# ndlongvn/MM-DTI

Measured on AMD Instinct MI355X. Metric: molecules/sec fwd+bwd (InfoNCE fine-tune), higher is better.
Workload: dtype fp16 forward / bf16 backward GEMM operands, fp32 accumulation

## Files before the change

### mm-dti_amd/csrc/pair_attn.h

```cpp
#pragma once
#include <type_traits>

#include "common.h"

namespace mmdti {

constexpr int HD = 8;

__device__ __forceinline__ void load8_bf16(const bf16_t* p, float (&o)[8]) {
  uint4 u = *reinterpret_cast<const uint4*>(p);
  uint32_t w[4] = {u.x, u.y, u.z, u.w};
#pragma unroll
  for (int i = 0; i < 4; ++i) {
    o[2 * i] = __uint_as_float(w[i] << 16);
    o[2 * i + 1] = __uint_as_float(w[i] & 0xffff0000u);
  }
}
__device__ __forceinline__ void store8_bf16(bf16_t* p, const float (&v)[8]) {
  uint4 u;
  u.x = (uint32_t)f2bf(v[0]) | ((uint32_t)f2bf(v[1]) << 16);
  u.y = (uint32_t)f2bf(v[2]) | ((uint32_t)f2bf(v[3]) << 16);
  u.z = (uint32_t)f2bf(v[4]) | ((uint32_t)f2bf(v[5]) << 16);
  u.w = (uint32_t)f2bf(v[6]) | ((uint32_t)f2bf(v[7]) << 16);
  *reinterpret_cast<uint4*>(p) = u;
}


typedef float f32x4 __attribute__((ext_vector_type(4)));

typedef short pa_s16x4 __attribute__((ext_vector_type(4)));
typedef __bf16 pa_bf16x4 __attribute__((ext_vector_type(4)));
typedef __attribute__((address_space(3))) pa_s16x4 pa_lds_s16x4;

__device__ __forceinline__ pa_s16x4 pa_pack4(const f32x4& v) {
  pa_bf16x4 h;
  h[0] = (__bf16)v[0]; h[1] = (__bf16)v[1]; h[2] = (__bf16)v[2]; h[3] = (__bf16)v[3];
  return __builtin_bit_cast(pa_s16x4, h);
}
__device__ __forceinline__ void pa_split4(const f32x4& v, pa_s16x4& hi, pa_s16x4& lo) {
  pa_bf16x4 h;
  h[0] = (__bf16)v[0]; h[1] = (__bf16)v[1]; h[2] = (__bf16)v[2]; h[3] = (__bf16)v[3];
  f32x4 r;
  r[0] = v[0] - (float)h[0]; r[1] = v[1] - (float)h[1]; r[2] = v[2] - (float)h[2]; r[3] = v[3] - (float)h[3];
  hi = __builtin_bit_cast(pa_s16x4, h);
  lo = pa_pack4(r);
}
#define PA_MFMA16(A, B, C) __builtin_amdgcn_mfma_f32_16x16x16bf16_1k(A, B, C, 0, 0, 0)
typedef _Float16 pa_h16x4 __attribute__((ext_vector_type(4)));
template <bool F16>
__device__ __forceinline__ f32x4 pa_mfma16(const pa_s16x4& a, const pa_s16x4& b, const f32x4& c) {
  if constexpr (F16) return __builtin_amdgcn_mfma_f32_16x16x16f16(__builtin_bit_cast(pa_h16x4, a), __builtin_bit_cast(pa_h16x4, b), c, 0, 0, 0);
  else return __builtin_amdgcn_mfma_f32_16x16x16bf16_1k(a, b, c, 0, 0, 0);
}
template <bool F16>
__device__ __forceinline__ void pa_split4_t(const f32x4& v, pa_s16x4& hi, pa_s16x4& lo) {
  if constexpr (F16) {
    pa_h16x4 h, l;
#pragma unroll
    for (int r = 0; r < 4; ++r) {
      h[r] = (_Float16)v[r];
      l[r] = (_Float16)(v[r] - (float)h[r]);
    }
    hi = __builtin_bit_cast(pa_s16x4, h);
    lo = __builtin_bit_cast(pa_s16x4, l);
  } else {
    pa_split4(v, hi, lo);
  }
}
#define PA_LOG2E 1.44269504088896340736f

typedef _Float16 pa_f16x4 __attribute__((ext_vector_type(4)));
__device__ __forceinline__ f32x4 pa_load4(const float* p) { return *reinterpret_cast<const f32x4*>(p); }
__device__ __forceinline__ f32x4 pa_load4_nt(const float* p) { return __builtin_nontemporal_load(reinterpret_cast<const f32x4*>(p)); }
__device__ __forceinline__ void pa_store4_nt(float* p, f32x4 v) { __builtin_nontemporal_store(v, reinterpret_cast<f32x4*>(p)); }
__device__ __forceinline__ f32x4 pa_round4(f32x4& keep, f32x4 v) { keep = v; return v; }

__device__ __forceinline__ f32x4 pa_widen_f16(const pa_f16x4& h) {
  f32x4 v;
#pragma unroll
  for (int r = 0; r < 4; ++r) v[r] = (float)h[r];
  return v;
}
__device__ __forceinline__ pa_f16x4 pa_narrow_f16(const f32x4& v) {
  pa_f16x4 h;
#pragma unroll
  for (int r = 0; r < 4; ++r) h[r] = (_Float16)v[r];
  return h;
}
__device__ __forceinline__ f32x4 pa_load4(const _Float16* p) { return pa_widen_f16(*reinterpret_cast<const pa_f16x4*>(p)); }
__device__ __forceinline__ f32x4 pa_load4_nt(const _Float16* p) { return pa_widen_f16(__builtin_nontemporal_load(reinterpret_cast<const pa_f16x4*>(p))); }
__device__ __forceinline__ void pa_store4_nt(_Float16* p, const f32x4& v) {
  __builtin_nontemporal_store(pa_narrow_f16(v), reinterpret_cast<pa_f16x4*>(p));
}
__device__ __forceinline__ f32x4 pa_round4(pa_f16x4& keep, const f32x4& v) {
  f32x4 c;
#pragma unroll
  for (int r = 0; r < 4; ++r) c[r] = __builtin_amdgcn_fmed3f(v[r], -INFINITY, 65504.f);
  keep = pa_narrow_f16(c);
  return pa_widen_f16(keep);
}
__device__ __forceinline__ void pa_store4_nt(_Float16* p, const pa_f16x4& h) { __builtin_nontemporal_store(h, reinterpret_cast<pa_f16x4*>(p)); }

__device__ __forceinline__ f32x4 pa_widen_bf16(const pa_s16x4& h) {
  f32x4 v;
#pragma unroll
  for (int r = 0; r < 4; ++r) v[r] = __builtin_bit_cast(float, (uint32_t)(uint16_t)h[r] << 16);
  return v;
}
__device__ __forceinline__ f32x4 pa_load4(const __bf16* p) { return pa_widen_bf16(*reinterpret_cast<const pa_s16x4*>(p)); }
__device__ __forceinline__ f32x4 pa_load4_nt(const __bf16* p) { return pa_widen_bf16(__builtin_nontemporal_load(reinterpret_cast<const pa_s16x4*>(p))); }
__device__ __forceinline__ void pa_store4_nt(__bf16* p, const f32x4& v) { __builtin_nontemporal_store(pa_pack4(v), reinterpret_cast<pa_s16x4*>(p)); }

__host__ __device__ constexpr int pa_kt_step(int nt) { return nt <= 9 ? 1 : (nt <= 13 ? 2 : 4); }
__host__ __device__ constexpr int pa_kt_effective(int kt, int nt) {
  const int s = pa_kt_step(nt), k = ((kt < 1 ? 1 : kt) + s - 1) / s * s;
  return k >= nt ? nt : k;
}
template <int NT, int K, typename F>
__device__ __forceinline__ void pa_dispatch_kt(int ke, F&& f) {
  constexpr int step = pa_kt_step(NT);
  constexpr int below = (K == NT) ? ((NT - 1) / step) * step : K - step;
  if constexpr (below < 1) {
    f(std::integral_constant<int, K>{});
  } else {
    if (ke >= K) f(std::integral_constant<int, K>{});
    else pa_dispatch_kt<NT, below>(ke, f);
  }
}

}

#define PA_MAX_NT 17

static inline int check_common(const char* fn, int B, int N, int H, int ld) {
  MMDTI_REQUIRE(B > 0 && N > 0 && H > 0, "%s: B,N,H must be positive", fn);
  MMDTI_REQUIRE(N <= 320, "%s: N=%d exceeds the supported 320 atoms (+BOS/EOS)", fn, N);
  MMDTI_REQUIRE(ld >= N, "%s: ld (%d) < N (%d)", fn, ld, N);
  MMDTI_REQUIRE((long long)B * H <= 2147483647LL, "%s: grid too large", fn);
  return MMDTI_OK;
}
```

### mm-dti_amd/csrc/pair_attn.hip

```cpp
#include "pair_attn.h"

namespace mmdti {

template <int NCH>
__global__ __launch_bounds__(256) void pair_attn_fwd_kernel(const bf16_t* __restrict__ qkv,
                                                            const float* __restrict__ bias_in,
                                                            float* __restrict__ s_out, bf16_t* __restrict__ o,
                                                            const unsigned char* __restrict__ key_pad, int N, int H,
                                                            int ld, float scale, uint32_t thresh, float dscale,
                                                            uint64_t seed, uint32_t site) {
  __shared__ __attribute__((aligned(16))) float sq[NCH * 64][HD];
  const int bh = xcd_chunk(blockIdx.x, gridDim.x), b = bh / H, h = bh - b * H;
  const int D = H * HD, D3 = 3 * D;
  const int tid = threadIdx.x, lane = tid & 63, wave = tid >> 6;
  const bf16_t* base = qkv + (long long)b * N * D3 + h * HD;
  for (int t = tid; t < N; t += 256) {
    float q[8];
    load8_bf16(base + (long long)t * D3, q);
#pragma unroll
    for (int d = 0; d < 8; ++d) sq[t][d] = q[d];
  }
  float k[NCH][8], v[NCH][8];
  bool masked[NCH];
#pragma unroll
  for (int c = 0; c < NCH; ++c) {
    const int j = c * 64 + lane;
    masked[c] = true;
#pragma unroll
    for (int d = 0; d < 8; ++d) k[c][d] = v[c][d] = 0.f;
    if (j < N) {
      load8_bf16(base + (long long)j * D3 + D, k[c]);
      load8_bf16(base + (long long)j * D3 + 2 * D, v[c]);
      masked[c] = key_pad ? key_pad[b * N + j] != 0 : false;
    }
  }
  __syncthreads();
  const float NEG_INF = -INFINITY;
  float nb[NCH];
#pragma unroll
  for (int c = 0; c < NCH; ++c) {
    const int j = c * 64 + lane;
    nb[c] = (wave < N && j < N && !masked[c]) ? bias_in[((long long)bh * N + wave) * ld + j] : 0.f;
  }
  for (int i = wave; i < N; i += 4) {
    const float4 q0 = *reinterpret_cast<const float4*>(&sq[i][0]);
    const float4 q1 = *reinterpret_cast<const float4*>(&sq[i][4]);
    const long long rowoff = ((long long)bh * N + i) * ld;
    float cb[NCH];
#pragma unroll
    for (int c = 0; c < NCH; ++c) cb[c] = nb[c];
    if (i + 4 < N) {
#pragma unroll
      for (int c = 0; c < NCH; ++c) {
        const int j = c * 64 + lane;
        nb[c] = (j < N && !masked[c]) ? bias_in[rowoff + 4LL * ld + j] : 0.f;
      }
    }
    float sv[NCH];
    float m = NEG_INF;
#pragma unroll
    for (int c = 0; c < NCH; ++c) {
      const int j = c * 64 + lane;
      float s = NEG_INF;
      if (j < N) {
        float dot = q0.x * k[c][0] + q0.y * k[c][1] + q0.z * k[c][2] + q0.w * k[c][3] + q1.x * k[c][4] +
                    q1.y * k[c][5] + q1.z * k[c][6] + q1.w * k[c][7];
        s = masked[c] ? NEG_INF : scale * dot + cb[c];
        s_out[rowoff + j] = s;
      }
      sv[c] = s;
      m = fmaxf(m, s);
    }
    m = wave_max(m);
    float sum = 0.f;
#pragma unroll
    for (int c = 0; c < NCH; ++c) {
      sv[c] = __expf(sv[c] - m);
      sum += sv[c];
    }
    const float inv = 1.0f / wave_sum(sum);
    float acc[8] = {0.f, 0.f, 0.f, 0.f, 0.f, 0.f, 0.f, 0.f};
#pragma unroll
    for (int c = 0; c < NCH; ++c) {
      float p = sv[c] * inv;
      if (thresh) {
        const int j = c * 64 + lane;
        bool keep = dropout_keep(seed, site, ((uint64_t)bh * N + i) * ld + j, thresh);
        p = keep ? p * dscale : 0.f;
      }
#pragma unroll
      for (int d = 0; d < 8; ++d) acc[d] += p * v[c][d];
    }
    const float tot = wave_sum8_scatter(acc, lane);
    if (lane < 8) o[((long long)b * N + i) * D + h * HD + lane] = f2bf(tot);
  }
}

template <int NT, bool TILED, bool FULL, bool RAG, typename ST, bool F16 = false>
__global__ __launch_bounds__(256, NT > 9 ? 2 : 4) void pair_attn_fwd_mfma_kernel(const bf16_t* __restrict__ qkv, const ST* __restrict__ bias_in,
                                                                 ST* __restrict__ s_out, bf16_t* __restrict__ o,
                                                                 const unsigned char* __restrict__ key_pad, int N, int H, int ld,
                                                                 float scale, uint32_t thresh, float dscale, uint64_t seed,
                                                                 uint32_t site, const int* __restrict__ key_tiles, int rag_store,
                                                                 const int* __restrict__ row_off) {
  static_assert(TILED || sizeof(ST) == 4, "compact pair tensors exist in the tiled layout only");
  static_assert(!RAG || sizeof(ST) == 2, "key-tile skipping is built for the compact layout only");
  constexpr int NP = NT * 16;
  constexpr int KSTR = NP + 8;
  __shared__ __attribute__((aligned(16))) bf16_t sQ[NP * 8];
  __shared__ __attribute__((aligned(16))) bf16_t sK[NP * 8];
  __shared__ __attribute__((aligned(16))) bf16_t sVT[8 * KSTR];
  __shared__ __attribute__((aligned(16))) float sM[NP];
  const int bh = xcd_chunk(blockIdx.x, gridDim.x), b = bh / H, h = bh - b * H;
  const int D = H * HD, D3 = 3 * D;
  const int tid = threadIdx.x, lane = tid & 63, wave = tid >> 6, nwaves = blockDim.x >> 6;
  const int nKB = (N + 15) >> 4;
  const int kt = RAG ? pa_kt_effective(min(__builtin_amdgcn_readfirstlane(key_tiles[b]), nKB), NT) : NT;
  const bool packed = RAG && row_off != nullptr;
  const int row0 = packed ? __builtin_amdgcn_readfirstlane(row_off[b]) : b * N;
  const int rows = packed ? __builtin_amdgcn_readfirstlane(row_off[b + 1]) - row0 : N;
  const bf16_t* base = qkv + (long long)row0 * D3 + h * HD;
  for (int t = tid; t < NP; t += blockDim.x) {
    uint4 q = make_uint4(0u, 0u, 0u, 0u), kk = q, vv = q;
    float msk = 1.f;
    if (t < rows) {
      q = *reinterpret_cast<const uint4*>(base + (long long)t * D3);
      kk = *reinterpret_cast<const uint4*>(base + (long long)t * D3 + D);
      vv = *reinterpret_cast<const uint4*>(base + (long long)t * D3 + 2 * D);
      msk = (key_pad && key_pad[row0 + t]) ? 1.f : 0.f;
    }
    *reinterpret_cast<uint4*>(sQ + t * 8) = q;
    *reinterpret_cast<uint4*>(sK + t * 8) = kk;
    const uint32_t vw[4] = {vv.x, vv.y, vv.z, vv.w};
#pragma unroll
    for (int d = 0; d < 8; ++d) sVT[d * KSTR + t] = (bf16_t)((d & 1) ? (vw[d >> 1] >> 16) : (vw[d >> 1] & 0xffffu));
    sM[t] = msk;
  }
  for (int t = tid; t < 8 * 8; t += blockDim.x) sVT[(t >> 3) * KSTR + NP + (t & 7)] = 0;
  __syncthreads();
  const int g = lane >> 4, c16 = lane & 15;
  const float NEG_INF = -INFINITY;
  const int nlast = nKB - 1;
  const bool colok = 4 * g < N - 16 * nlast;
  const Rng24 rk = rng24_key(seed, site, (uint32_t)bh);
  auto body = [&](int qb, auto edge_c, auto kt_c) {
    constexpr bool EDGE = decltype(edge_c)::value;
    constexpr int KT = decltype(kt_c)::value;
    const int qi = qb * 16 + c16;
    const uint32_t t8 = thresh ? rng24_row_t8(rk, (uint32_t)qi, thresh) : 0u;
    const bool qvalid = EDGE ? qi < rows : true;
    const long long rowoff = ((long long)bh * N + (qvalid ? qi : 0)) * ld;
    const pa_s16x4 zero4 = {0, 0, 0, 0};
    const pa_s16x4 qv = g < 2 ? *reinterpret_cast<const pa_s16x4*>(sQ + (qb * 16 + c16) * 8 + 4 * g) : zero4;
    const int vr = EDGE ? min(16, N - qb * 16) : 16;
    const long long tbase = (long long)bh * pair_plane(N) + (long long)qb * 16 * pair_n4(N) + ((4 * g < pair_n4(N) ? g : 0) * vr + (qvalid ? c16 : 0)) * 4;
    const ST* bin = bias_in + (TILED ? tbase : rowoff);
    ST* sout = s_out + (TILED ? tbase : rowoff);
    const int TSTEP = TILED ? (EDGE ? vr * 16 : 256) : 16;
    const int goff = TILED ? 0 : 4 * g;
#define PA_PRED(T) (!TILED ? (qvalid && (T) * 16 + 4 * g < N) \
                           : (qvalid && (FULL ? ((T) < NT - 1 || colok) : ((T) < nlast || ((T) == nlast && colok)))))
#define PA_FAST(T) (TILED && !EDGE && (FULL ? (T) < NT - 1 : false))
    const float fillv = (TILED && qvalid) ? -INFINITY : 0.f;
    f32x4 S[KT];
#pragma unroll
    for (int t = 0; t < KT; ++t) {
      if (PA_FAST(t)) {
        S[t] = pa_load4_nt(bin + t * TSTEP + goff);
      } else {
        const bool pr = PA_PRED(t);
        const f32x4 ld4 = pa_load4(bin + (pr ? t * TSTEP + goff : 0));
        S[t] = pr ? ld4 : f32x4{fillv, fillv, fillv, fillv};
      }
    }
    float m = NEG_INF;
    if (RAG && rag_store) {
      const f32x4 ninf = {NEG_INF, NEG_INF, NEG_INF, NEG_INF};
#pragma unroll
      for (int t = KT; t < NT; ++t) {
        if (PA_FAST(t)) {
          pa_store4_nt(sout + t * TSTEP + goff, ninf);
        } else if (PA_PRED(t)) {
          pa_store4_nt(sout + t * TSTEP + goff, ninf);
        }
      }
    }
#pragma unroll
    for (int t = 0; t < KT; ++t) {
      {
        const int kcol = t * 16 + 4 * g;
        f32x4 c = S[t];
        const pa_s16x4 ka = g < 2 ? *reinterpret_cast<const pa_s16x4*>(sK + (t * 16 + c16) * 8 + 4 * g) : zero4;
        f32x4 qk = {0.f, 0.f, 0.f, 0.f};
        qk = pa_mfma16<F16>(ka, qv, qk);
#pragma unroll
        for (int r = 0; r < 4; ++r) c[r] += scale * qk[r];
        if (!TILED || key_pad) {
          const f32x4 km = *reinterpret_cast<const f32x4*>(&sM[kcol]);
#pragma unroll
          for (int r = 0; r < 4; ++r) c[r] = (km[r] != 0.f) ? NEG_INF : c[r];
        }
        typename std::conditional<sizeof(ST) == 2, pa_f16x4, f32x4>::type cs;
        c = pa_round4(cs, c);
        if (PA_FAST(t)) {
          pa_store4_nt(sout + t * TSTEP + goff, cs);
        } else if (PA_PRED(t)) {
          pa_store4_nt(sout + t * TSTEP + goff, cs);
        }
        S[t] = c;
        m = fmaxf(fmaxf(m, c[0]), c[1]);
        m = fmaxf(fmaxf(m, c[2]), c[3]);
      }
    }
    m = fmaxf(m, __shfl_xor(m, 16, 64));
    m = fmaxf(m, __shfl_xor(m, 32, 64));
    const float mneg = -m * PA_LOG2E;
    float lsum = 0.f;
#pragma unroll
    for (int t = 0; t < KT; ++t) {
      {
#pragma unroll
        for (int r = 0; r < 4; ++r) {
          const float e = __builtin_amdgcn_exp2f(fmaf(S[t][r], PA_LOG2E, mneg));
          S[t][r] = e;
          lsum += e;
        }
      }
    }
    lsum += __shfl_xor(lsum, 16, 64);
    lsum += __shfl_xor(lsum, 32, 64);
    const float inv = dscale / lsum;
    f32x4 oacc = {0.f, 0.f, 0.f, 0.f};
#pragma unroll
    for (int t = 0; t < KT; ++t) {
      {
        f32x4 p = S[t] * inv;
        if (thresh) {
          const uint32_t kw = rng24_word(rk, ((uint32_t)qi * (uint32_t)ld + t * 16 + 4 * g) >> 2);
#pragma unroll
          for (int r = 0; r < 4; ++r) p[r] = rng24_kept(kw, r, t8) ? p[r] : 0.f;
        }
        const pa_s16x4 va = *reinterpret_cast<const pa_s16x4*>(sVT + (c16 & 7) * KSTR + t * 16 + 4 * g);
        pa_s16x4 ph, pl;
        pa_split4_t<F16>(p, ph, pl);
        oacc = pa_mfma16<F16>(va, ph, oacc);
        oacc = pa_mfma16<F16>(va, pl, oacc);
      }
    }
    if (qvalid && g < 2) {
      uint2 pk;
      if constexpr (F16) {
        pk.x = f2h_sat2(oacc[0], oacc[1]);
        pk.y = f2h_sat2(oacc[2], oacc[3]);
      } else {
        pk.x = (uint32_t)f2bf(oacc[0]) | ((uint32_t)f2bf(oacc[1]) << 16);
        pk.y = (uint32_t)f2bf(oacc[2]) | ((uint32_t)f2bf(oacc[3]) << 16);
      }
      *reinterpret_cast<uint2*>(o + ((long long)row0 + qi) * D + h * HD + 4 * g) = pk;
    }
#undef PA_PRED
#undef PA_FAST
  };
  const int nQB = packed ? (rows + 15) >> 4 : nKB;
  auto run = [&](auto kt_c) {
    for (int qb = wave; qb < nQB; qb += nwaves) {
      if (TILED && qb * 16 + 16 <= rows) body(qb, std::false_type{}, kt_c);
      else body(qb, std::true_type{}, kt_c);
    }
  };
  if constexpr (RAG) pa_dispatch_kt<NT, NT>(kt, run);
  else run(std::integral_constant<int, NT>{});
}


}
MMDTI_DEFINE_SALT_PULL(pair_attn)
using namespace mmdti;

extern "C" int mmdti_pair_attn_fwd(mmdti_stream_t stream, const void* qkv_bf16, const void* bias_in, void* s_out,
                                   void* o_bf16, const unsigned char* key_pad, int B, int N, int H, int ld,
                                   float scale, float drop_p, unsigned long long seed, unsigned int site, int layout,
                                   const int* key_tiles, int rag_store, const int* row_off, int qkv_f16) {
  const int tiled = layout & 1, compact = (layout >> 1) & 1;
  if (int e = check_common("pair_attn_fwd", B, N, H, ld)) return e;
  MMDTI_REQUIRE((layout & ~3) == 0 && (!compact || tiled), "pair_attn_fwd: layout must be 0 (row-major fp32), 1 (tiled fp32) or 3 (tiled, fp16 logits)");
  MMDTI_REQUIRE(!key_tiles || compact, "pair_attn_fwd: key_tiles (ragged batches) needs the compact tiled pair layout (layout 3)");
  MMDTI_REQUIRE(!row_off || key_tiles, "pair_attn_fwd: packed token rows (row_off) need key_tiles");
  MMDTI_REQUIRE(!qkv_f16 || compact, "pair_attn_fwd: fp16 q | k | v (the fp16 forward-operand mode) is built for the compact tiled pair layout (layout 3)");
  MMDTI_REQUIRE(!tiled || (ld % 4 == 0 && N <= 16 * PA_MAX_NT), "pair_attn_fwd: the tiled pair layout needs ld %% 4 == 0 and N <= 272");
  MMDTI_REQUIRE(qkv_bf16 && bias_in && s_out && o_bf16, "pair_attn_fwd: null pointer");
  MMDTI_REQUIRE(aligned16(qkv_bf16), "pair_attn_fwd: qkv must be 16-byte aligned");
  MMDTI_REQUIRE(!tiled || (aligned16(bias_in) && aligned16(s_out)), "pair_attn_fwd: tiled pair tensors must be 16-byte aligned");
  MMDTI_REQUIRE(drop_p >= 0.f && drop_p < 1.f, "pair_attn_fwd: dropout p out of range");
  const uint32_t th = dropout_thresh(drop_p);
  const uint32_t th8 = dropout_thresh8(drop_p);
  const float sc = drop_p > 0.f ? 1.f / (1.f - drop_p) : 1.f;
  dim3 grid(B * H), block(256);
  hipStream_t s = (hipStream_t)stream;
  if (ld % 4 == 0 && aligned16(bias_in) && aligned16(s_out) && N <= 16 * PA_MAX_NT) {
    const int nqb = (N + 15) / 16;
    dim3 blk(nqb % 3 == 0 ? 192 : (nqb < 4 ? 64 * nqb : 256));
#define PA_M(NT, TL, FL, RG, ST)                                                                                                     \
  hipLaunchKernelGGL((pair_attn_fwd_mfma_kernel<NT, TL, FL, RG, ST>), grid, blk, 0, s, (const bf16_t*)qkv_bf16, (const ST*)bias_in, \
                     (ST*)s_out, (bf16_t*)o_bf16, key_pad, N, H, ld, scale, th8, sc, (uint64_t)seed, (uint32_t)site, key_tiles, rag_store, row_off)
#define PA_MT(NT)                                                                           \
  do {                                                                                      \
    if (!tiled) PA_M(NT, false, false, false, float);                                       \
    else if (!compact) { if (nqb == NT) PA_M(NT, true, true, false, float); else PA_M(NT, true, false, false, float); } \
  } while (0)
#define PA_MH(NT, RG)                                                                                                                  \
  hipLaunchKernelGGL((pair_attn_fwd_mfma_kernel<NT, true, true, RG, _Float16, true>), grid, blk, 0, s, (const bf16_t*)qkv_bf16,       \
                     (const _Float16*)bias_in, (_Float16*)s_out, (bf16_t*)o_bf16, key_pad, N, H, ld, scale, th8, sc, (uint64_t)seed,  \
                     (uint32_t)site, key_tiles, rag_store, row_off)
#define PA_MC(NT) case NT: if (qkv_f16) { if (key_tiles) PA_MH(NT, true); else PA_MH(NT, false); } \
                           else if (key_tiles) PA_M(NT, true, true, true, _Float16); else PA_M(NT, true, true, false, _Float16); break
    if (compact) {
      switch (nqb) {
        PA_MC(1); PA_MC(2); PA_MC(3); PA_MC(4); PA_MC(5); PA_MC(6); PA_MC(7); PA_MC(8); PA_MC(9); PA_MC(10); PA_MC(11); PA_MC(12);
        PA_MC(13); PA_MC(14); PA_MC(15); PA_MC(16); PA_MC(17);
      }
    } else if (nqb <= 5) PA_MT(5); else if (nqb <= 9) PA_MT(9); else if (nqb <= 13) PA_MT(13); else PA_MT(17);
#undef PA_MC
#undef PA_MH
#undef PA_MT
#undef PA_M
    MMDTI_LAUNCH_CHECK();
    return MMDTI_OK;
  }
#define PA_F(NCH)                                                                                                   \
  hipLaunchKernelGGL((pair_attn_fwd_kernel<NCH>), grid, block, 0, s, (const bf16_t*)qkv_bf16, (const float*)bias_in, (float*)s_out, \
                     (bf16_t*)o_bf16, key_pad, N, H, ld, scale, th, sc, (uint64_t)seed, (uint32_t)site)
  switch ((N + 63) / 64) {
    case 1: PA_F(1); break;
    case 2: PA_F(2); break;
    case 3: PA_F(3); break;
    case 4: PA_F(4); break;
    default: PA_F(5); break;
  }
#undef PA_F
  MMDTI_LAUNCH_CHECK();
  return MMDTI_OK;
}
```

### mm-dti_amd/csrc/pair_attn_bwd_mfma.h

```cpp
#pragma once
#include "pair_attn.h"

namespace mmdti {

template <int NT, bool TILED, bool FULL, int NW, bool RAG, typename ST, typename GT>
__global__ __launch_bounds__(64 * NW, NT > 9 ? ((NT >= 16 && NW == 3) ? 2 : 1) : 3) void pair_attn_bwd_mfma_kernel(const bf16_t* __restrict__ qkv, const ST* __restrict__ s_in,
                                                                 const bf16_t* __restrict__ dO, const GT* __restrict__ gin, GT* __restrict__ gout,
                                                                 bf16_t* __restrict__ dqkv, int N, int H, int ld, float scale,
                                                                 int g_in_zero, uint32_t thresh, float dscale, uint64_t seed,
                                                                 uint32_t site, const int* __restrict__ key_tiles,
                                                                 const int* __restrict__ row_off, int qkv_f16) {
  static_assert(TILED || (sizeof(ST) == 4 && sizeof(GT) == 4), "compact pair tensors exist in the tiled layout only");
  static_assert(!RAG || sizeof(ST) == 2, "key-tile skipping is built for the compact layout only");
  constexpr int NP = NT * 16;
  constexpr int KSTR = NP + 8;
  __shared__ __attribute__((aligned(16))) bf16_t sQ[NP * 8 + 16];
  __shared__ __attribute__((aligned(16))) bf16_t sD[NP * 8 + 16];
  __shared__ __attribute__((aligned(16))) bf16_t sV[NP * 8];
  __shared__ __attribute__((aligned(16))) bf16_t sKT[8 * KSTR];
  __shared__ __attribute__((aligned(16))) float redw[NW * NT * 2 * 128];
  __shared__ __attribute__((aligned(16))) bf16_t patch[NW][2][256];
  const int bh = xcd_chunk(blockIdx.x, gridDim.x), b = bh / H, h = bh - b * H;
  const int D = H * HD, D3 = 3 * D;
  const int tid = threadIdx.x, lane = tid & 63, wave = tid >> 6, nwaves = blockDim.x >> 6;
  const int nKB = (N + 15) >> 4;
  const int kt = RAG ? pa_kt_effective(min(__builtin_amdgcn_readfirstlane(key_tiles[b]), nKB), NT) : NT;
  const bool packed = RAG && row_off != nullptr;
  const int row0 = packed ? __builtin_amdgcn_readfirstlane(row_off[b]) : b * N;
  const int rows = packed ? __builtin_amdgcn_readfirstlane(row_off[b + 1]) - row0 : N;
  const bf16_t* base = qkv + (long long)row0 * D3 + h * HD;
  for (int t = tid; t < NP + 2; t += blockDim.x) {
    uint4 q = make_uint4(0u, 0u, 0u, 0u), kk = q, vv = q, dd = q;
    if (t < rows) {
      q = *reinterpret_cast<const uint4*>(base + (long long)t * D3);
      kk = *reinterpret_cast<const uint4*>(base + (long long)t * D3 + D);
      vv = *reinterpret_cast<const uint4*>(base + (long long)t * D3 + 2 * D);
      dd = *reinterpret_cast<const uint4*>(dO + ((long long)row0 + t) * D + h * HD);
      if (qkv_f16) { q = h2bf8(q); kk = h2bf8(kk); vv = h2bf8(vv); }
    }
    *reinterpret_cast<uint4*>(sQ + t * 8) = q;
    *reinterpret_cast<uint4*>(sD + t * 8) = dd;
    if (t < NP) {
      *reinterpret_cast<uint4*>(sV + t * 8) = vv;
      const uint32_t kw[4] = {kk.x, kk.y, kk.z, kk.w};
#pragma unroll
      for (int d = 0; d < 8; ++d) sKT[d * KSTR + t] = (bf16_t)((d & 1) ? (kw[d >> 1] >> 16) : (kw[d >> 1] & 0xffffu));
    }
  }
  for (int t = tid; t < 8 * 8; t += blockDim.x) sKT[(t >> 3) * KSTR + NP + (t & 7)] = 0;
  for (int t = tid; t < NW * NT * 2 * 128; t += blockDim.x) redw[t] = 0.f;
  __syncthreads();
  const int g = lane >> 4, c16 = lane & 15;
  const bool dlane = c16 < 8;
  const float NEG_INF = -INFINITY;
  bf16_t* pw = &patch[wave][0][0];
  const int pwr = c16 * 16 + ((g ^ ((c16 >> 3) << 1)) << 2);
  const int prd = (4 * g + (c16 >> 2)) * 16 + (((c16 & 3) ^ ((g >> 1) << 1)) << 2);
  const pa_s16x4 zero4 = {0, 0, 0, 0};
  const int nlast = nKB - 1;
  const bool colok = 4 * g < N - 16 * nlast;
  const Rng24 rk = rng24_key(seed, site, (uint32_t)bh);
  auto body = [&](int qb, auto edge_c, auto kt_c) {
    constexpr bool EDGE = decltype(edge_c)::value;
    constexpr int KT = decltype(kt_c)::value;
    const int qi = qb * 16 + c16;
    const uint32_t t8 = thresh ? rng24_row_t8(rk, (uint32_t)qi, thresh) : 0u;
    const bool qvalid = EDGE ? qi < rows : true;
    const long long rowoff = ((long long)bh * N + (qvalid ? qi : 0)) * ld;
    const int vr = EDGE ? min(16, N - qb * 16) : 16;
    const long long tbase = (long long)bh * pair_plane(N) + (long long)qb * 16 * pair_n4(N) + ((4 * g < pair_n4(N) ? g : 0) * vr + (qvalid ? c16 : 0)) * 4;
    const ST* sin_p = s_in + (TILED ? tbase : rowoff);
    const GT* gin_p = gin + (TILED ? tbase : rowoff);
    GT* gout_p = gout + (TILED ? tbase : rowoff);
    const int TSTEP = TILED ? (EDGE ? vr * 16 : 256) : 16;
    const int goff = TILED ? 0 : 4 * g;
#define PA_PRED(T) (!TILED ? (qvalid && (T) * 16 + 4 * g < N) \
                           : (qvalid && (FULL ? ((T) < NT - 1 || colok) : ((T) < nlast || ((T) == nlast && colok)))))
#define PA_FAST(T) (TILED && !EDGE && (FULL ? (T) < NT - 1 : false))
    const pa_s16x4 dob = g < 2 ? *reinterpret_cast<const pa_s16x4*>(sD + (qb * 16 + c16) * 8 + 4 * g) : zero4;
    const int trq = (qb * 16 + 4 * g + (c16 >> 2)) * 8 + 4 * (c16 & 3);
    const pa_s16x4 bD = __builtin_amdgcn_ds_read_tr16_b64_v4i16((pa_lds_s16x4*)(sD + trq));
    const pa_s16x4 bQ = __builtin_amdgcn_ds_read_tr16_b64_v4i16((pa_lds_s16x4*)(sQ + trq));
    f32x4 P[KT];
    float m = NEG_INF;
#pragma unroll
    for (int t = 0; t < KT; ++t) {
      {
        const int kcol = t * 16 + 4 * g;
        f32x4 c;
        if (PA_FAST(t)) {
          c = pa_load4_nt(sin_p + t * TSTEP + goff);
        } else {
          const bool inrow = PA_PRED(t);
          const f32x4 ld4 = pa_load4(sin_p + (inrow ? t * TSTEP + goff : 0));
          c = inrow ? ld4 : f32x4{NEG_INF, NEG_INF, NEG_INF, NEG_INF};
        }
        if (!TILED) {
#pragma unroll
          for (int r = 0; r < 4; ++r) c[r] = (kcol + r < N) ? c[r] : NEG_INF;
        }
        P[t] = c;
        m = fmaxf(fmaxf(m, c[0]), c[1]);
        m = fmaxf(fmaxf(m, c[2]), c[3]);
      }
    }
    m = fmaxf(m, __shfl_xor(m, 16, 64));
    m = fmaxf(m, __shfl_xor(m, 32, 64));
    if (m == NEG_INF) m = 0.f;
    const float mneg = -m * PA_LOG2E;
    float lsum = 0.f;
#pragma unroll
    for (int t = 0; t < KT; ++t) {
      {
#pragma unroll
        for (int r = 0; r < 4; ++r) {
          const float e = __builtin_amdgcn_exp2f(fmaf(P[t][r], PA_LOG2E, mneg));
          P[t][r] = e;
          lsum += e;
        }
      }
    }
    lsum += __shfl_xor(lsum, 16, 64);
    lsum += __shfl_xor(lsum, 32, 64);
    const float inv = lsum > 0.f ? 1.0f / lsum : 0.f;
    float dl = 0.f;
#pragma unroll
    for (int t = 0; t < KT; ++t) {
      {
        const pa_s16x4 va = g < 2 ? *reinterpret_cast<const pa_s16x4*>(sV + (t * 16 + c16) * 8 + 4 * g) : zero4;
        f32x4 dp = {0.f, 0.f, 0.f, 0.f};
        dp = PA_MFMA16(va, dob, dp);
        f32x4 pr = P[t] * inv;
        if (thresh) {
          const uint32_t kw = rng24_word(rk, ((uint32_t)qi * (uint32_t)ld + t * 16 + 4 * g) >> 2);
#pragma unroll
          for (int r = 0; r < 4; ++r) {
            const bool kp = rng24_kept(kw, r, t8);
            dp[r] = kp ? dp[r] * dscale : 0.f;
            dl += dp[r] * pr[r];
            pr[r] = kp ? pr[r] : -pr[r];
          }
        } else {
          dl += dp[0] * pr[0] + dp[1] * pr[1] + dp[2] * pr[2] + dp[3] * pr[3];
        }
        P[t] = pr;
      }
    }
    dl += __shfl_xor(dl, 16, 64);
    dl += __shfl_xor(dl, 32, 64);
    constexpr int PA_LA = 3;
    auto load_gin = [&](int t) -> f32x4 {
      if (PA_FAST(t)) {
        const f32x4 ld4 = pa_load4_nt(gin_p + (g_in_zero ? 0 : t * TSTEP + goff));
        return g_in_zero ? f32x4{0.f, 0.f, 0.f, 0.f} : ld4;
      }
      const bool inrow = PA_PRED(t) && !g_in_zero;
      const f32x4 ld4 = pa_load4(gin_p + (inrow ? t * TSTEP + goff : 0));
      return inrow ? ld4 : f32x4{0.f, 0.f, 0.f, 0.f};
    };
    f32x4 Gq[PA_LA];
#pragma unroll
    for (int t = 0; t < PA_LA && t < KT; ++t) Gq[t] = load_gin(t);
    f32x4 dq = {0.f, 0.f, 0.f, 0.f};
    const int dcol = dlane ? c16 : 0;
#pragma unroll
    for (int t = 0; t < KT; ++t) {
      const int kcol = t * 16 + 4 * g;
      const f32x4 Gin = Gq[t % PA_LA];
      if (t + PA_LA < KT) Gq[t % PA_LA] = load_gin(t + PA_LA);
      __builtin_amdgcn_sched_barrier(0);
      const pa_s16x4 va = g < 2 ? *reinterpret_cast<const pa_s16x4*>(sV + (t * 16 + c16) * 8 + 4 * g) : zero4;
      f32x4 dp = {0.f, 0.f, 0.f, 0.f};
      dp = PA_MFMA16(va, dob, dp);
      f32x4 G;
#pragma unroll
      for (int r = 0; r < 4; ++r) G[r] = fabsf(P[t][r]) * ((P[t][r] > 0.f ? dp[r] * dscale : 0.f) - dl) + Gin[r];
      if (!TILED && t * 16 + 16 > N) {
#pragma unroll
        for (int r = 0; r < 4; ++r) G[r] = (kcol + r < N) ? G[r] : 0.f;
      }
      if (EDGE && !qvalid) G = f32x4{0.f, 0.f, 0.f, 0.f};
      if (PA_FAST(t)) {
        pa_store4_nt(gout_p + t * TSTEP + goff, G);
      } else if (PA_PRED(t)) {
        pa_store4_nt(gout_p + t * TSTEP + goff, G);
      }
      f32x4 Pd;
#pragma unroll
      for (int r = 0; r < 4; ++r) Pd[r] = P[t][r] > 0.f ? P[t][r] * dscale : 0.f;
      if (EDGE && !qvalid) Pd = f32x4{0.f, 0.f, 0.f, 0.f};
      pa_s16x4 Gh, Gl, Ph, Pl;
      pa_split4(G, Gh, Gl);
      pa_split4(Pd, Ph, Pl);
      *reinterpret_cast<pa_s16x4*>(pw + pwr) = Ph;
      *reinterpret_cast<pa_s16x4*>(pw + 256 + pwr) = Gh;
      const pa_s16x4 ka = *reinterpret_cast<const pa_s16x4*>(sKT + (c16 & 7) * KSTR + t * 16 + 4 * g);
      dq = PA_MFMA16(ka, Gh, dq);
      dq = PA_MFMA16(ka, Gl, dq);
      __builtin_amdgcn_fence(__ATOMIC_RELEASE, "wavefront");
      __builtin_amdgcn_wave_barrier();
      __builtin_amdgcn_fence(__ATOMIC_ACQUIRE, "wavefront");
      const pa_s16x4 aPh = __builtin_amdgcn_ds_read_tr16_b64_v4i16((pa_lds_s16x4*)(pw + prd));
      const pa_s16x4 aGh = __builtin_amdgcn_ds_read_tr16_b64_v4i16((pa_lds_s16x4*)(pw + 256 + prd));
      __builtin_amdgcn_fence(__ATOMIC_RELEASE, "wavefront");
      __builtin_amdgcn_wave_barrier();
      __builtin_amdgcn_fence(__ATOMIC_ACQUIRE, "wavefront");
      *reinterpret_cast<pa_s16x4*>(pw + pwr) = Pl;
      *reinterpret_cast<pa_s16x4*>(pw + 256 + pwr) = Gl;
      __builtin_amdgcn_fence(__ATOMIC_RELEASE, "wavefront");
      __builtin_amdgcn_wave_barrier();
      __builtin_amdgcn_fence(__ATOMIC_ACQUIRE, "wavefront");
      const pa_s16x4 aPl = __builtin_amdgcn_ds_read_tr16_b64_v4i16((pa_lds_s16x4*)(pw + prd));
      const pa_s16x4 aGl = __builtin_amdgcn_ds_read_tr16_b64_v4i16((pa_lds_s16x4*)(pw + 256 + prd));
      float* accK = redw + ((wave * NT + t) * 2 + 0) * 128 + (g * 8 + dcol) * 4;
      float* accV = accK + 128;
      f32x4 dKt = *reinterpret_cast<const f32x4*>(accK), dVt = *reinterpret_cast<const f32x4*>(accV);
      dVt = PA_MFMA16(aPh, bD, dVt);
      dKt = PA_MFMA16(aGh, bQ, dKt);
      dVt = PA_MFMA16(aPl, bD, dVt);
      dKt = PA_MFMA16(aGl, bQ, dKt);
      if (dlane) {
        *reinterpret_cast<f32x4*>(accK) = dKt;
        *reinterpret_cast<f32x4*>(accV) = dVt;
      }
      __builtin_amdgcn_fence(__ATOMIC_RELEASE, "wavefront");
      __builtin_amdgcn_wave_barrier();
      __builtin_amdgcn_fence(__ATOMIC_ACQUIRE, "wavefront");
    }
    if (qvalid && g < 2) {
      uint2 pk;
      pk.x = (uint32_t)f2bf(dq[0] * scale) | ((uint32_t)f2bf(dq[1] * scale) << 16);
      pk.y = (uint32_t)f2bf(dq[2] * scale) | ((uint32_t)f2bf(dq[3] * scale) << 16);
      *reinterpret_cast<uint2*>(dqkv + ((long long)row0 + qi) * D3 + h * HD + 4 * g) = pk;
    }
#undef PA_PRED
#undef PA_FAST
  };
  const int nQB = packed ? (rows + 15) >> 4 : nKB;
  auto run = [&](auto kt_c) {
    for (int qb = wave; qb < nQB; qb += nwaves) {
      if (TILED && qb * 16 + 16 <= rows) body(qb, std::false_type{}, kt_c);
      else body(qb, std::true_type{}, kt_c);
    }
  };
  if constexpr (RAG) pa_dispatch_kt<NT, NT>(kt, run);
  else run(std::integral_constant<int, NT>{});
  __syncthreads();
  for (int key = tid; key < rows; key += blockDim.x) {
    const int t = key >> 4, kg = (key & 15) >> 2, r = key & 3;
    float a[8] = {0, 0, 0, 0, 0, 0, 0, 0}, c2[8] = {0, 0, 0, 0, 0, 0, 0, 0};
    for (int w = 0; w < nwaves; ++w) {
      const float* bk = redw + ((w * NT + t) * 2) * 128 + kg * 32 + r;
#pragma unroll
      for (int d = 0; d < 8; ++d) {
        a[d] += bk[d * 4];
        c2[d] += bk[128 + d * 4];
      }
    }
#pragma unroll
    for (int d = 0; d < 8; ++d) a[d] *= scale;
    bf16_t* dst = dqkv + ((long long)row0 + key) * D3 + h * HD;
    store8_bf16(dst + D, a);
    store8_bf16(dst + 2 * D, c2);
  }
}


template <typename GT>
static inline void pa_bwd_compact_launch(int nqb, dim3 grid, dim3 blk, hipStream_t st, const void* qkv_bf16, const void* s, const void* do_bf16,
                                         void* g, void* dqkv_bf16, int N, int H, int ld, float scale, int g_in_zero, uint32_t th8, float sc,
                                         unsigned long long seed, unsigned int site, const int* key_tiles, const int* row_off, int qkv_f16) {
#define PA_MBH(NT, NWV, RG)                                                                                                   \
  hipLaunchKernelGGL((pair_attn_bwd_mfma_kernel<NT, true, true, NWV, RG, _Float16, GT>), grid, blk, 0, st, (const bf16_t*)qkv_bf16, \
                     (const _Float16*)s, (const bf16_t*)do_bf16, (const GT*)g, (GT*)g, (bf16_t*)dqkv_bf16, N, H, ld, scale,    \
                     g_in_zero, th8, sc, (uint64_t)seed, (uint32_t)site, key_tiles, row_off, qkv_f16)
#define PA_MBC(NT)                                                                                   \
  case NT:                                                                                           \
    if (key_tiles) PA_MBH(NT, ((NT % 3 == 0 || NT >= 16 || NT == 5) ? 3 : 4), true);                 \
    else PA_MBH(NT, ((NT % 3 == 0 || NT >= 16 || NT == 5) ? 3 : 4), false);                          \
    break
  switch (nqb) {
    PA_MBC(1); PA_MBC(2); PA_MBC(3); PA_MBC(4); PA_MBC(5); PA_MBC(6); PA_MBC(7); PA_MBC(8); PA_MBC(9); PA_MBC(10); PA_MBC(11);
    PA_MBC(12); PA_MBC(13); PA_MBC(14); PA_MBC(15); PA_MBC(16); PA_MBC(17);
  }
#undef PA_MBC
#undef PA_MBH
}
void pa_bwd_compact_launch_g16(int nqb, dim3 grid, dim3 blk, hipStream_t st, const void* qkv_bf16, const void* s, const void* do_bf16, void* g,
                               void* dqkv_bf16, int N, int H, int ld, float scale, int g_in_zero, uint32_t th8, float sc,
                               unsigned long long seed, unsigned int site, const int* key_tiles, const int* row_off, int qkv_f16);

}
```

Measured before the change: 4899.

## Keep compact fp16 pair scores packed in forward softmax and streamline conversions

In the forward pair-attention kernel, scores in the compact fp16 layout are now held as packed half vectors. The key-pad mask becomes an fp16 clamp applied with packed min, and the row max is taken with packed max, replacing the per-element fp32 select and fmed3 clamp. The K tile in shared memory is doubled with a zero half, so the MFMA operand load no longer branches on lane group. The dropout branch is hoisted out of the P·V loop via a compile-time flag. bf16/fp16 split helpers now use vector conversions and an fma_mix inline-asm residual, and the backward kernel skips the gin load when g_in_zero is set. Together these cut VALU work and registers but add inline asm and more shared memory.

```diff
diff --git a/mm-dti_amd/csrc/pair_attn.h b/mm-dti_amd/csrc/pair_attn.h
--- a/mm-dti_amd/csrc/pair_attn.h
+++ b/mm-dti_amd/csrc/pair_attn.h
@@ -32,18 +32,18 @@
 typedef __bf16 pa_bf16x4 __attribute__((ext_vector_type(4)));
 typedef __attribute__((address_space(3))) pa_s16x4 pa_lds_s16x4;
 
+typedef float pa_f32x2 __attribute__((ext_vector_type(2)));
+typedef __bf16 pa_bf16x2 __attribute__((ext_vector_type(2)));
 __device__ __forceinline__ pa_s16x4 pa_pack4(const f32x4& v) {
-  pa_bf16x4 h;
-  h[0] = (__bf16)v[0]; h[1] = (__bf16)v[1]; h[2] = (__bf16)v[2]; h[3] = (__bf16)v[3];
-  return __builtin_bit_cast(pa_s16x4, h);
+  const uint2 u = {__builtin_bit_cast(uint32_t, __builtin_convertvector(pa_f32x2{v[0], v[1]}, pa_bf16x2)),
+                   __builtin_bit_cast(uint32_t, __builtin_convertvector(pa_f32x2{v[2], v[3]}, pa_bf16x2))};
+  return __builtin_bit_cast(pa_s16x4, u);
 }
 __device__ __forceinline__ void pa_split4(const f32x4& v, pa_s16x4& hi, pa_s16x4& lo) {
-  pa_bf16x4 h;
-  h[0] = (__bf16)v[0]; h[1] = (__bf16)v[1]; h[2] = (__bf16)v[2]; h[3] = (__bf16)v[3];
-  f32x4 r;
-  r[0] = v[0] - (float)h[0]; r[1] = v[1] - (float)h[1]; r[2] = v[2] - (float)h[2]; r[3] = v[3] - (float)h[3];
-  hi = __builtin_bit_cast(pa_s16x4, h);
-  lo = pa_pack4(r);
+  hi = pa_pack4(v);
+  const uint2 u = __builtin_bit_cast(uint2, hi);
+  const f32x4 h = {__uint_as_float(u.x << 16), __uint_as_float(u.x & 0xffff0000u), __uint_as_float(u.y << 16), __uint_as_float(u.y & 0xffff0000u)};
+  lo = pa_pack4(v - h);
 }
 #define PA_MFMA16(A, B, C) __builtin_amdgcn_mfma_f32_16x16x16bf16_1k(A, B, C, 0, 0, 0)
 typedef _Float16 pa_h16x4 __attribute__((ext_vector_type(4)));
@@ -52,17 +52,22 @@
   if constexpr (F16) return __builtin_amdgcn_mfma_f32_16x16x16f16(__builtin_bit_cast(pa_h16x4, a), __builtin_bit_cast(pa_h16x4, b), c, 0, 0, 0);
   else return __builtin_amdgcn_mfma_f32_16x16x16bf16_1k(a, b, c, 0, 0, 0);
 }
+__device__ __forceinline__ f32x4 pa_residual_f16(const f32x4& v, const pa_h16x4& h) {
+  const uint2 w = __builtin_bit_cast(uint2, h);
+  f32x4 d;
+  asm("v_fma_mix_f32 %0, %1, -1.0, %2 op_sel_hi:[1,0,0]" : "=v"(d[0]) : "v"(w.x), "v"(v[0]));
+  asm("v_fma_mix_f32 %0, %1, -1.0, %2 op_sel:[1,0,0] op_sel_hi:[1,0,0]" : "=v"(d[1]) : "v"(w.x), "v"(v[1]));
+  asm("v_fma_mix_f32 %0, %1, -1.0, %2 op_sel_hi:[1,0,0]" : "=v"(d[2]) : "v"(w.y), "v"(v[2]));
+  asm("v_fma_mix_f32 %0, %1, -1.0, %2 op_sel:[1,0,0] op_sel_hi:[1,0,0]" : "=v"(d[3]) : "v"(w.y), "v"(v[3]));
+  return d;
+}
 template <bool F16>
 __device__ __forceinline__ void pa_split4_t(const f32x4& v, pa_s16x4& hi, pa_s16x4& lo) {
   if constexpr (F16) {
-    pa_h16x4 h, l;
-#pragma unroll
-    for (int r = 0; r < 4; ++r) {
-      h[r] = (_Float16)v[r];
-      l[r] = (_Float16)(v[r] - (float)h[r]);
-    }
+    const pa_h16x4 h = __builtin_convertvector(v, pa_h16x4);
+    const f32x4 d = pa_residual_f16(v, h);
     hi = __builtin_bit_cast(pa_s16x4, h);
-    lo = __builtin_bit_cast(pa_s16x4, l);
+    lo = __builtin_bit_cast(pa_s16x4, __builtin_convertvector(d, pa_h16x4));
   } else {
     pa_split4(v, hi, lo);
   }
@@ -73,7 +78,6 @@
 __device__ __forceinline__ f32x4 pa_load4(const float* p) { return *reinterpret_cast<const f32x4*>(p); }
 __device__ __forceinline__ f32x4 pa_load4_nt(const float* p) { return __builtin_nontemporal_load(reinterpret_cast<const f32x4*>(p)); }
 __device__ __forceinline__ void pa_store4_nt(float* p, f32x4 v) { __builtin_nontemporal_store(v, reinterpret_cast<f32x4*>(p)); }
-__device__ __forceinline__ f32x4 pa_round4(f32x4& keep, f32x4 v) { keep = v; return v; }
 
 __device__ __forceinline__ f32x4 pa_widen_f16(const pa_f16x4& h) {
   f32x4 v;
@@ -92,14 +96,25 @@
 __device__ __forceinline__ void pa_store4_nt(_Float16* p, const f32x4& v) {
   __builtin_nontemporal_store(pa_narrow_f16(v), reinterpret_cast<pa_f16x4*>(p));
 }
-__device__ __forceinline__ f32x4 pa_round4(pa_f16x4& keep, const f32x4& v) {
-  f32x4 c;
-#pragma unroll
-  for (int r = 0; r < 4; ++r) c[r] = __builtin_amdgcn_fmed3f(v[r], -INFINITY, 65504.f);
-  keep = pa_narrow_f16(c);
-  return pa_widen_f16(keep);
+__device__ __forceinline__ void pa_store4_nt(_Float16* p, const pa_f16x4& h) { __builtin_nontemporal_store(h, reinterpret_cast<pa_f16x4*>(p)); }
+__device__ __forceinline__ f32x4 pa_load4s(const float* p) { return pa_load4(p); }
+__device__ __forceinline__ f32x4 pa_load4s_nt(const float* p) { return pa_load4_nt(p); }
+__device__ __forceinline__ pa_f16x4 pa_load4s(const _Float16* p) { return *reinterpret_cast<const pa_f16x4*>(p); }
+__device__ __forceinline__ pa_f16x4 pa_load4s_nt(const _Float16* p) { return __builtin_nontemporal_load(reinterpret_cast<const pa_f16x4*>(p)); }
+__device__ __forceinline__ pa_f16x4 pa_pk_min4(const pa_f16x4& a, const pa_f16x4& b) {
+  const uint2 x = __builtin_bit_cast(uint2, a), y = __builtin_bit_cast(uint2, b);
+  uint2 d;
+  asm("v_pk_min_f16 %0, %1, %2" : "=v"(d.x) : "v"(x.x), "v"(y.x));
+  asm("v_pk_min_f16 %0, %1, %2" : "=v"(d.y) : "v"(x.y), "v"(y.y));
+  return __builtin_bit_cast(pa_f16x4, d);
 }
-__device__ __forceinline__ void pa_store4_nt(_Float16* p, const pa_f16x4& h) { __builtin_nontemporal_store(h, reinterpret_cast<pa_f16x4*>(p)); }
+__device__ __forceinline__ pa_f16x4 pa_pk_max4(const pa_f16x4& a, const pa_f16x4& b) {
+  const uint2 x = __builtin_bit_cast(uint2, a), y = __builtin_bit_cast(uint2, b);
+  uint2 d;
+  asm("v_pk_max_f16 %0, %1, %2" : "=v"(d.x) : "v"(x.x), "v"(y.x));
+  asm("v_pk_max_f16 %0, %1, %2" : "=v"(d.y) : "v"(x.y), "v"(y.y));
+  return __builtin_bit_cast(pa_f16x4, d);
+}
 
 __device__ __forceinline__ f32x4 pa_widen_bf16(const pa_s16x4& h) {
   f32x4 v;
diff --git a/mm-dti_amd/csrc/pair_attn.hip b/mm-dti_amd/csrc/pair_attn.hip
--- a/mm-dti_amd/csrc/pair_attn.hip
+++ b/mm-dti_amd/csrc/pair_attn.hip
@@ -108,9 +108,11 @@
   constexpr int NP = NT * 16;
   constexpr int KSTR = NP + 8;
   __shared__ __attribute__((aligned(16))) bf16_t sQ[NP * 8];
-  __shared__ __attribute__((aligned(16))) bf16_t sK[NP * 8];
+  __shared__ __attribute__((aligned(16))) bf16_t sK[2 * NP * 8];
   __shared__ __attribute__((aligned(16))) bf16_t sVT[8 * KSTR];
-  __shared__ __attribute__((aligned(16))) float sM[NP];
+  constexpr bool CST = sizeof(ST) == 2;
+  typedef typename std::conditional<CST, _Float16, float>::type MT;
+  __shared__ __attribute__((aligned(16))) MT sM[NP];
   const int bh = xcd_chunk(blockIdx.x, gridDim.x), b = bh / H, h = bh - b * H;
   const int D = H * HD, D3 = 3 * D;
   const int tid = threadIdx.x, lane = tid & 63, wave = tid >> 6, nwaves = blockDim.x >> 6;
@@ -122,19 +124,21 @@
   const bf16_t* base = qkv + (long long)row0 * D3 + h * HD;
   for (int t = tid; t < NP; t += blockDim.x) {
     uint4 q = make_uint4(0u, 0u, 0u, 0u), kk = q, vv = q;
-    float msk = 1.f;
+    bool msk = true;
     if (t < rows) {
       q = *reinterpret_cast<const uint4*>(base + (long long)t * D3);
       kk = *reinterpret_cast<const uint4*>(base + (long long)t * D3 + D);
       vv = *reinterpret_cast<const uint4*>(base + (long long)t * D3 + 2 * D);
-      msk = (key_pad && key_pad[row0 + t]) ? 1.f : 0.f;
+      msk = key_pad && key_pad[row0 + t];
     }
     *reinterpret_cast<uint4*>(sQ + t * 8) = q;
     *reinterpret_cast<uint4*>(sK + t * 8) = kk;
+    *reinterpret_cast<uint4*>(sK + NP * 8 + t * 8) = make_uint4(0u, 0u, 0u, 0u);
     const uint32_t vw[4] = {vv.x, vv.y, vv.z, vv.w};
 #pragma unroll
     for (int d = 0; d < 8; ++d) sVT[d * KSTR + t] = (bf16_t)((d & 1) ? (vw[d >> 1] >> 16) : (vw[d >> 1] & 0xffffu));
-    sM[t] = msk;
+    if constexpr (CST) sM[t] = (key_pad && msk) ? (_Float16)-INFINITY : (_Float16)65504.f;
+    else sM[t] = msk ? 1.f : 0.f;
   }
   for (int t = tid; t < 8 * 8; t += blockDim.x) sVT[(t >> 3) * KSTR + NP + (t & 7)] = 0;
   __syncthreads();
@@ -143,6 +147,8 @@
   const int nlast = nKB - 1;
   const bool colok = 4 * g < N - 16 * nlast;
   const Rng24 rk = rng24_key(seed, site, (uint32_t)bh);
+  const bf16_t* kap = sK + (g < 2 ? 0 : NP * 8) + c16 * 8 + 4 * (g & 1);
+  typedef typename std::conditional<CST, pa_f16x4, f32x4>::type SQ;
   auto body = [&](int qb, auto edge_c, auto kt_c) {
     constexpr bool EDGE = decltype(edge_c)::value;
     constexpr int KT = decltype(kt_c)::value;
@@ -161,19 +167,21 @@
 #define PA_PRED(T) (!TILED ? (qvalid && (T) * 16 + 4 * g < N) \
                            : (qvalid && (FULL ? ((T) < NT - 1 || colok) : ((T) < nlast || ((T) == nlast && colok)))))
 #define PA_FAST(T) (TILED && !EDGE && (FULL ? (T) < NT - 1 : false))
-    const float fillv = (TILED && qvalid) ? -INFINITY : 0.f;
-    f32x4 S[KT];
+    typedef typename std::conditional<CST, _Float16, float>::type SE;
+    const SE fillv = (TILED && qvalid) ? (SE)-INFINITY : (SE)0.f;
+    SQ S[KT];
 #pragma unroll
     for (int t = 0; t < KT; ++t) {
       if (PA_FAST(t)) {
-        S[t] = pa_load4_nt(bin + t * TSTEP + goff);
+        S[t] = pa_load4s_nt(bin + t * TSTEP + goff);
       } else {
         const bool pr = PA_PRED(t);
-        const f32x4 ld4 = pa_load4(bin + (pr ? t * TSTEP + goff : 0));
-        S[t] = pr ? ld4 : f32x4{fillv, fillv, fillv, fillv};
+        const SQ ld4 = pa_load4s(bin + (pr ? t * TSTEP + goff : 0));
+        S[t] = pr ? ld4 : SQ{fillv, fillv, fillv, fillv};
       }
     }
     float m = NEG_INF;
+    pa_f16x4 mh = {(_Float16)-INFINITY, (_Float16)-INFINITY, (_Float16)-INFINITY, (_Float16)-INFINITY};
     if (RAG && rag_store) {
       const f32x4 ninf = {NEG_INF, NEG_INF, NEG_INF, NEG_INF};
 #pragma unroll
@@ -189,40 +197,51 @@
     for (int t = 0; t < KT; ++t) {
       {
         const int kcol = t * 16 + 4 * g;
-        f32x4 c = S[t];
-        const pa_s16x4 ka = g < 2 ? *reinterpret_cast<const pa_s16x4*>(sK + (t * 16 + c16) * 8 + 4 * g) : zero4;
+        const pa_s16x4 ka = *reinterpret_cast<const pa_s16x4*>(kap + t * 128);
         f32x4 qk = {0.f, 0.f, 0.f, 0.f};
         qk = pa_mfma16<F16>(ka, qv, qk);
-#pragma unroll
-        for (int r = 0; r < 4; ++r) c[r] += scale * qk[r];
-        if (!TILED || key_pad) {
-          const f32x4 km = *reinterpret_cast<const f32x4*>(&sM[kcol]);
-#pragma unroll
-          for (int r = 0; r < 4; ++r) c[r] = (km[r] != 0.f) ? NEG_INF : c[r];
-        }
-        typename std::conditional<sizeof(ST) == 2, pa_f16x4, f32x4>::type cs;
-        c = pa_round4(cs, c);
+        f32x4 c;
+#pragma unroll
+        for (int r = 0; r < 4; ++r) c[r] = (float)S[t][r] + scale * qk[r];
+        SQ cs;
+        if constexpr (CST) {
+          cs = __builtin_convertvector(c, pa_f16x4);
+          cs = pa_pk_min4(cs, *reinterpret_cast<const pa_f16x4*>(&sM[kcol]));
+          mh = pa_pk_max4(mh, cs);
+        } else {
+          if (!TILED || key_pad) {
+            const f32x4 km = *reinterpret_cast<const f32x4*>(&sM[kcol]);
+#pragma unroll
+            for (int r = 0; r < 4; ++r) c[r] = (km[r] != 0.f) ? NEG_INF : c[r];
+          }
+          cs = c;
+          m = fmaxf(fmaxf(m, c[0]), c[1]);
+          m = fmaxf(fmaxf(m, c[2]), c[3]);
+        }
         if (PA_FAST(t)) {
           pa_store4_nt(sout + t * TSTEP + goff, cs);
         } else if (PA_PRED(t)) {
           pa_store4_nt(sout + t * TSTEP + goff, cs);
         }
-        S[t] = c;
-        m = fmaxf(fmaxf(m, c[0]), c[1]);
-        m = fmaxf(fmaxf(m, c[2]), c[3]);
-      }
+        S[t] = cs;
+      }
+    }
+    if constexpr (CST) {
+      const _Float16 m01 = __builtin_elementwise_max(mh[0], mh[1]), m23 = __builtin_elementwise_max(mh[2], mh[3]);
+      m = (float)__builtin_elementwise_max(m01, m23);
     }
     m = fmaxf(m, __shfl_xor(m, 16, 64));
     m = fmaxf(m, __shfl_xor(m, 32, 64));
     const float mneg = -m * PA_LOG2E;
     float lsum = 0.f;
+    f32x4 E[KT];
 #pragma unroll
     for (int t = 0; t < KT; ++t) {
       {
 #pragma unroll
         for (int r = 0; r < 4; ++r) {
-          const float e = __builtin_amdgcn_exp2f(fmaf(S[t][r], PA_LOG2E, mneg));
-          S[t][r] = e;
+          const float e = __builtin_amdgcn_exp2f(fmaf((float)S[t][r], PA_LOG2E, mneg));
+          E[t][r] = e;
           lsum += e;
         }
       }
@@ -231,11 +250,11 @@
     lsum += __shfl_xor(lsum, 32, 64);
     const float inv = dscale / lsum;
     f32x4 oacc = {0.f, 0.f, 0.f, 0.f};
-#pragma unroll
-    for (int t = 0; t < KT; ++t) {
-      {
-        f32x4 p = S[t] * inv;
-        if (thresh) {
+    auto pv = [&](auto drop_c) {
+#pragma unroll
+      for (int t = 0; t < KT; ++t) {
+        f32x4 p = E[t] * inv;
+        if constexpr (decltype(drop_c)::value) {
           const uint32_t kw = rng24_word(rk, ((uint32_t)qi * (uint32_t)ld + t * 16 + 4 * g) >> 2);
 #pragma unroll
           for (int r = 0; r < 4; ++r) p[r] = rng24_kept(kw, r, t8) ? p[r] : 0.f;
@@ -246,7 +265,9 @@
         oacc = pa_mfma16<F16>(va, ph, oacc);
         oacc = pa_mfma16<F16>(va, pl, oacc);
       }
-    }
+    };
+    if (thresh) pv(std::true_type{});
+    else pv(std::false_type{});
     if (qvalid && g < 2) {
       uint2 pk;
       if constexpr (F16) {
diff --git a/mm-dti_amd/csrc/pair_attn_bwd_mfma.h b/mm-dti_amd/csrc/pair_attn_bwd_mfma.h
--- a/mm-dti_amd/csrc/pair_attn_bwd_mfma.h
+++ b/mm-dti_amd/csrc/pair_attn_bwd_mfma.h
@@ -151,8 +151,9 @@
     constexpr int PA_LA = 3;
     auto load_gin = [&](int t) -> f32x4 {
       if (PA_FAST(t)) {
-        const f32x4 ld4 = pa_load4_nt(gin_p + (g_in_zero ? 0 : t * TSTEP + goff));
-        return g_in_zero ? f32x4{0.f, 0.f, 0.f, 0.f} : ld4;
+        f32x4 ld4 = {0.f, 0.f, 0.f, 0.f};
+        if (!g_in_zero) ld4 = pa_load4_nt(gin_p + t * TSTEP + goff);
+        return ld4;
       }
       const bool inrow = PA_PRED(t) && !g_in_zero;
       const f32x4 ld4 = pa_load4(gin_p + (inrow ? t * TSTEP + goff : 0));
```

New measurement: 4947, median of 6. About the same (+1.0%).
